# antbern/slamrs

Hardware: NVIDIA B200
Metric: particle_beam_updates_per_s (higher is better)
Workload: dtype f32 geometry, f64 weights, u16x2 hit-counter cells

## Files before the change

slamrs_b200/csrc/api.cu:

```cuda
#include "../../include/slamrs_gpu.h"

#include <cuda_runtime.h>
#include <math.h>
#include <stdio.h>
#include <stdlib.h>
#include <string.h>
#include <unistd.h>

#include <algorithm>
#include <new>
#include <string>
#include <vector>

#include "comm.h"
#include "kernels.cuh"

using namespace slamrs;

struct slamrs_gpu_handle {
    slamrs_gpu_config cfg{};
    int device = 0;
    int num_sms = 148;
    cudaStream_t stream = nullptr;
    cudaStream_t side_stream = nullptr;
// ... 362 lines not shown
        launch_publish_counters(h->stream, h->d_counters, h->h_counters);
        h->launches++;
    }
    CU_TRY(h, cudaStreamSynchronize(h->stream));
    CU_TRY(h, cudaGetLastError());
    h->counters_fresh = true;
    return SLAMRS_OK;
}

int loc_step_async(slamrs_gpu_handle* h, const OdomModel& od, bool caller) {
    cudaStream_t s = h->stream;
    if (h->profiling && h->prof_recorded == PROF_RING) {
        int prc = prof_flush(h);
        if (prc) return prc;
    }
    const int cur = h->cur, nxt = cur ^ 1;
    const ScanDevice scan = h->scan_external ? ScanDevice{h->ext_angle, h->ext_dist, h->ext_valid, h->n_beams, nullptr}
                                             : ScanDevice{h->d_angle, h->d_dist, h->d_valid, h->n_beams, nullptr};
    PROF_MARK(h, 0);
    launch_loc_step(s, h->geom, od, scan, h->d_pose[cur], h->d_results, h->n_total, caller ? h->d_z : nullptr, h->cfg.seed,
                    h->step, h->d_loc_terms, h->loc_outside, h->d_carry, h->d_counters);
    PROF_MARK(h, 1);
    PROF_MARK(h, 2);
    launch_weights(s, h->d_results, h->n_total, h->d_wnorm, h->d_cum, h->d_fold, (double)h->cfg.resample_threshold, h->d_counters);
    launch_resample_indices(s, h->d_results, h->d_cum, h->n_total, caller ? h->d_u : nullptr, h->cfg.seed, h->step, h->d_idx,
                            h->d_pose[nxt], 0, h->n_total, false, nullptr,
                            RayLists{nullptr, nullptr, nullptr, nullptr, nullptr, nullptr, 0u, 0u}, h->d_wnorm, h->d_carry,
                            h->d_counters);
    h->launches += 3;
    for (uint32_t m = 3; m < PROF_MARKS; ++m) PROF_MARK(h, m);
    if (h->profiling) h->prof_recorded++;
    CU_TRY(h, cudaGetLastError());
    h->cur = nxt;
    h->step++;
    h->counters_fresh = false;
    h->mirror_by_step = false;
    return SLAMRS_OK;
}

}

namespace {
template <typename T>
struct DevBuf {
    T* p = nullptr;
    cudaError_t alloc(size_t n) { return cudaMalloc(&p, sizeof(T) * (n ? n : 1)); }
    ~DevBuf() { cudaFree(p); }
};
int debug_device(int device) {
    int n = 0;
    if (cudaGetDeviceCount(&n) != cudaSuccess || n == 0) { cudaGetLastError(); return SLAMRS_E_NO_DEVICE; }
// ... 506 lines not shown
    const bool flag_pulls = h->world > 1 && fuse && half_items && h->boxed_copy && h->p2p_exchange;
    const uint32_t pull_epoch = flag_pulls ? (uint32_t)(h->step + 1ull) : 0u;
    const size_t n_zero = half_items ? 2 * (size_t)h->n_slots + 2 * (size_t)h->n_local : 0;
    PROF_MARK(h, 0);
    launch_motion_likelihood(s, h->geom, od, scan, h->d_pose[cur], h->d_slot[cur], h->defer ? h->d_alias : nullptr, h->d_cells, h->d_meta, h->cells_per_grid,
                             h->d_results, h->first, h->n_local, caller ? h->d_z : nullptr, h->cfg.seed, h->step, h->d_term_table, h->d_valid_list, h->d_n_valid,
                             h->d_carry, h->d_counters, h->p2p_exchange ? h->d_peer_results : nullptr, res_off, h->rank, h->world,
                             h->d_readers, (uint32_t)n_zero, h->match_on ? &h->match : nullptr, h->d_match_stats);
    h->launches += h->match_on ? 3 : 2;
    h->match_last_step = h->match_on;
    h->match_last_max_moves = h->match.max_moves;
    PROF_MARK(h, 1);
    if (h->world > 1) {
        if (h->p2p_exchange) {
            int brc = step_barrier(h);
            if (brc) return brc;
        } else {
            std::string err;
            if (comm_all_gather(h->comm, h->d_results + h->first, h->d_results, sizeof(ParticleResult) * h->n_local, s, &err))
                return fail(h, SLAMRS_E_NCCL, err);
        }
    }
    PROF_MARK(h, 2);
    launch_weights(s, h->d_results, h->n_total, h->d_wnorm, h->d_cum, h->d_fold, (double)h->cfg.resample_threshold, h->d_counters);
    RayLists ray{nullptr, nullptr, nullptr, nullptr, nullptr, nullptr, 0u, 0u};
    if (fuse) ray = RayLists{h->d_ray_items, h->d_ray_items + h->n_local, h->d_slot[cur], h->d_alias, h->d_readers, h->d_meta,
                             h->n_local, flag_pulls ? 1u : 0u};
    launch_resample_indices(s, h->d_results, h->d_cum, h->n_total, caller ? h->d_u : nullptr, h->cfg.seed, h->step,
                            h->d_idx, h->d_pose[nxt], h->first, h->n_local, !all_particles, h->d_alive, ray, h->d_wnorm, h->d_carry,
                            h->d_counters);
    if (all_particles) {
        launch_mark_alive(s, h->d_idx, h->n_total, h->first, h->n_local, true, h->d_alive, h->d_counters);
        h->launches++;
    }
    if (h->defer && !fuse) {
        if (all_particles)
            launch_materialize_list(s, nullptr, h->n_total, h->first, h->n_local, h->d_slot[cur], h->d_alias, h->d_cells,
                                    h->cells_per_grid, h->d_meta, h->d_bands, h->n_bands, h->d_mat_items, h->d_mat_leaders,
                                    h->d_mat_roots, h->d_counters);
        else
            launch_materialize_alive(s, h->d_alive, h->n_local, h->d_slot[cur], h->d_alias, h->d_cells, h->cells_per_grid,
                                     h->d_meta, h->d_bands, h->n_bands, h->d_mat_items, h->d_counters);
        h->launches++;
    }
    CU_TRY(h, cudaEventRecord(h->ev_indices, s));
    CU_TRY(h, cudaStreamWaitEvent(h->side_stream, h->ev_indices, 0));
    PlanArgs pa{};
    pa.results = h->d_results;
    pa.idx = h->d_idx;
    pa.n_total = h->n_total; pa.n_local = h->n_local; pa.rank = h->rank; pa.world = h->world;
    pa.slot_old = h->d_slot[cur]; pa.slot_new = h->d_slot[nxt];
    pa.keep = h->d_keep; pa.need = h->d_need; pa.free_list = h->d_free; pa.spare_list = h->d_spare;
    pa.n_spare_cap = h->n_spare;
    pa.copies = h->d_copies; pa.leaders = h->d_leaders;
    pa.cells = h->d_cells; pa.cells_per_grid = h->cells_per_grid;
    pa.peer_cells = h->d_peer_cells;
    pa.meta = h->d_meta; pa.peer_meta = h->d_peer_meta;
    pa.bands = h->d_bands; pa.peer_bands = h->d_peer_bands; pa.n_bands = h->n_bands;
    pa.counters = h->d_counters;
    pa.history = h->d_history;
    pa.step = h->step;
    pa.staged = plan_can_stage(h->n_local, h->n_spare);
    pa.alias_of = h->d_alias; pa.defer = h->defer;
    launch_plan(h->side_stream, pa);
    h->launches += 3;
    if (flag_pulls) {
        launch_pull(h->side_stream, h->d_copies, h->d_leaders, &h->d_counters->n_copies, &h->d_counters->n_leaders,
                    h->n_local, h->geom, h->d_counters, h->num_sms, pull_epoch, h->barrier_timeout_ns, h->d_meta, h->d_readers,
                    h->d_readers + h->n_slots);
        h->launches++;
    }
    CU_TRY(h, cudaEventRecord(h->ev_plan, h->side_stream));
    PROF_MARK(h, 3);
    if (h->defer && !fuse) {
        int mrc = materialize_copies(h, all_particles);
        if (mrc) return mrc;
    }
    PROF_MARK(h, 4);
    if (h->order_pending) {
        CU_TRY(h, cudaStreamWaitEvent(s, h->ev_sort, 0));
        h->order_pending = false;
    }
    CU_TRY(h, launch_ray_update(s, h->geom, scan, h->d_results, h->first, h->n_local, h->d_alive,
                                fuse ? h->d_ray_items : nullptr, fuse ? h->d_ray_items + h->n_local : nullptr,
                                fuse ? h->d_readers : nullptr,
                                fuse ? h->d_readers + h->n_slots : nullptr, h->d_readers + 2 * (size_t)h->n_slots, h->d_ray_xchg,
                                h->d_ray_spill, h->d_slot[cur],
                                h->d_cells, h->d_meta, h->d_bands, h->cells_per_grid, h->radius_cells, h->d_counters, &h->window_cells,
// ... 566 lines not shown
                                       uint64_t out_shape[4]) {
    if (!raw_weights || !out_idx || n == 0 || n > 0x7fffffffu || !(tau >= 0.0 && tau <= 1.0)) return SLAMRS_E_INVALID_ARG;
    int rc = debug_device(device);
    if (rc) return rc;
    DeviceGuard g(device < 0 ? 0 : device);
    DBG_CU(configure_kernels());
    DevBuf<ParticleResult> res;
    DevBuf<double> wn, cum, fold, u;
    DevBuf<uint32_t> idx;
    DevBuf<StepCounters> cnt;
    DBG_CU(res.alloc(n)); DBG_CU(wn.alloc(n)); DBG_CU(cum.alloc(n)); DBG_CU(fold.alloc(weights_scratch_doubles()));
    DBG_CU(u.alloc(1)); DBG_CU(idx.alloc(n)); DBG_CU(cnt.alloc(1));
    std::vector<ParticleResult> host(n);
    for (uint32_t i = 0; i < n; ++i) { host[i].weight = raw_weights[i]; host[i].x = host[i].y = host[i].theta = 0.0f; host[i].slot = 0; }
    DBG_CU(cudaMemcpy(res.p, host.data(), sizeof(ParticleResult) * (size_t)n, cudaMemcpyHostToDevice));
    DBG_CU(cudaMemcpy(u.p, &u01, sizeof(double), cudaMemcpyHostToDevice));
    DBG_CU(cudaMemset(cnt.p, 0, sizeof(StepCounters)));
    cudaEvent_t ev[3];
    for (auto& e : ev) DBG_CU(cudaEventCreate(&e));
    const int reps = out_us ? 20 : 1;
    float us[2] = {0.f, 0.f};
    for (int r = 0; r < reps; ++r) {
        cudaEventRecord(ev[0], nullptr);
        launch_weights(nullptr, res.p, n, wn.p, cum.p, fold.p, tau, cnt.p);
        cudaEventRecord(ev[1], nullptr);
        launch_resample_indices(nullptr, res.p, cum.p, n, u.p, 0, 0, idx.p, nullptr, 0, 0, false, nullptr,
                                RayLists{nullptr, nullptr, nullptr, nullptr, nullptr, nullptr, 0u, 0u}, wn.p, nullptr, cnt.p);
        cudaEventRecord(ev[2], nullptr);
        cudaError_t e = cudaDeviceSynchronize();
        if (e != cudaSuccess) { for (auto& x : ev) cudaEventDestroy(x); return fail(nullptr, SLAMRS_E_CUDA, cudaGetErrorString(e)); }
        float a = 0.f, b = 0.f;
        cudaEventElapsedTime(&a, ev[0], ev[1]); cudaEventElapsedTime(&b, ev[1], ev[2]);
        if (r > 0 || reps == 1) { us[0] += a * 1000.f; us[1] += b * 1000.f; }
    }
    for (auto& e : ev) cudaEventDestroy(e);
    if (out_us) { out_us[0] = us[0] / (float)(reps > 1 ? reps - 1 : 1); out_us[1] = us[1] / (float)(reps > 1 ? reps - 1 : 1); }
    StepCounters c;
    DBG_CU(cudaMemcpy(&c, cnt.p, sizeof(c), cudaMemcpyDeviceToHost));
    DBG_CU(cudaMemcpy(out_idx, idx.p, sizeof(uint32_t) * (size_t)n, cudaMemcpyDeviceToHost));
    if (out_norm) DBG_CU(cudaMemcpy(out_norm, wn.p, sizeof(double) * (size_t)n, cudaMemcpyDeviceToHost));
    if (out_cum) DBG_CU(cudaMemcpy(out_cum, cum.p, sizeof(double) * (size_t)n, cudaMemcpyDeviceToHost));
    if (out_max_particle) *out_max_particle = c.max_particle;
    if (out_us && getenv("SLAMRS_FOLD_TRACE_PRINT")) {
        long long tr[64];
        if (weights_trace(tr) == 0) {
            fprintf(stderr, "k_weights clock stamps (cycles from start):");
            for (int k = 0; k < 44; ++k) fprintf(stderr, " [%d]%lld", k, tr[k] ? tr[k] - tr[0] : -1);
            fprintf(stderr, "\n");
        }
    }
// ... 12 lines not shown
```

slamrs_b200/csrc/kernels.cuh:

```cuda
#pragma once
#include <cuda_runtime.h>
#include <stdint.h>
#include "slam_device.cuh"

namespace slamrs {

struct alignas(8) ParticleResult {
    double weight;
    float x, y, theta;
    int32_t slot;
};
static_assert(sizeof(ParticleResult) == 24, "ParticleResult is exchanged between GPUs as 24 bytes");

struct StepCounters {
    unsigned long long max_particle;
    unsigned long long n_copies;
    unsigned long long n_leaders;
    unsigned long long n_pulls;
    unsigned long long distinct;
    unsigned long long clamped;
    unsigned long long saturated;
    unsigned long long spilled;
    unsigned long long staging_short;
    long long est_slot;
// ... 115 lines not shown
                         uint32_t rank, uint32_t world, unsigned long long epoch, unsigned long long timeout_ns,
                         StepCounters* counters);
void launch_peer_goodbye(cudaStream_t stream, unsigned long long* const* peer_flags, unsigned long long* my_flags,
                         uint32_t rank, uint32_t world, unsigned long long timeout_ns, StepCounters* counters);

bool ray_update_can_fuse(const MapGeom& geom, uint32_t n_beams, size_t cells_per_grid, bool force_generic, int radius_cells);
size_t ray_spill_scratch_words(int num_sms);
size_t ray_half_xchg_bytes();
int ray_trace(unsigned long long* out18);
cudaError_t launch_ray_update(cudaStream_t stream, MapGeom geom, ScanDevice scan, const ParticleResult* results,
                              uint32_t first_particle, uint32_t n_local, const uint32_t* alive_list,
                              const RayItem* clones, const RayItem* owners, const uint32_t* readers, uint32_t* done,
                              uint32_t* xflag , void* xchg ,
                              uint32_t* spill_scratch,
                              const int32_t* slot_of, uint32_t* cells, SlotMeta* meta, uint32_t* bands,
                              size_t cells_per_grid, int radius_cells, StepCounters* counters,
                              uint64_t* window_cells, bool force_generic, int num_sms,
                              uint32_t* xdone ,

                              uint32_t signal_epoch );

struct WeightsShape { uint32_t cluster, threads, chunk; bool regs; };
WeightsShape weights_shape(uint32_t n_total);
void launch_weights(cudaStream_t stream, const ParticleResult* results, uint32_t n_total, double* w_norm,
                    double* cum, double* fold_scratch, double resample_tau, StepCounters* counters);
size_t weights_scratch_doubles();
int weights_trace(long long* out64);

void launch_resample_indices(cudaStream_t stream, const ParticleResult* results, const double* cum,
                             uint32_t n_total, const double* u01_caller, uint64_t seed, uint64_t step,
                             uint32_t* idx, float* pose_next, uint32_t first_particle, uint32_t n_local,
                             bool build_alive ,
                             uint32_t* alive_list, RayLists ray, const double* w_norm, double* carry ,
                             StepCounters* counters);

struct PlanArgs {
    const ParticleResult* results;
    const uint32_t* idx;
    uint32_t n_total, n_local, rank, world;
    const int32_t* slot_old;
    int32_t* slot_new;
    int32_t* keep;
    int32_t* need;
    int32_t* free_list;
    int32_t* spare_list;
    uint32_t n_spare_cap;
    CopyItem* copies;
    uint32_t* leaders;
    uint32_t* cells;
    size_t cells_per_grid;
    uint32_t* const* peer_cells;
    SlotMeta* meta;
    SlotMeta* const* peer_meta;
    uint32_t* bands;
    uint32_t* const* peer_bands;
    uint32_t n_bands;
    StepCounters* counters;
// ... 74 lines not shown
```

slamrs_b200/csrc/kernels_resample.cu:

```cuda
#include "kernels_common.cuh"

namespace slamrs {


constexpr int W_CLUSTER = 8;

constexpr uint32_t FOLD_HEADS_PER_CTA = 32;
constexpr uint32_t FOLD_HEADS_MAX = FOLD_HEADS_PER_CTA * W_CLUSTER;
constexpr uint32_t FOLD_STAGE = 2048;
constexpr int FOLD_MAX_ROUNDS = 4;
constexpr int FOLD_MARGIN_BITS = 40;
constexpr int FOLD_LREG = 16;
constexpr int FOLD_THREADS = 512;
constexpr int FOLD_GENERIC_THREADS = 1024;
constexpr uint32_t FOLD_MAX_CHUNKS = FOLD_GENERIC_THREADS * W_CLUSTER;

struct FoldTd {
    double d0, d1;
    uint32_t qc;
};
template <int LREG>
struct FoldRec {
    double d0, d1;
    uint32_t q_prev;
// ... 263 lines not shown
                if (C == 1u) sh.total = s;
                else for (uint32_t r = 0; r < C; ++r) *cluster.map_shared_rank(&sh.total, r) = s;
            }
        }
        FOLD_STAMP(tb + 5);
        __syncthreads();
        if (tid < C) {
            if (C == 1u) sh.cta_bad[0] = sh.bad;
            else cluster.map_shared_rank(&sh.cta_bad[0], tid)[crank] = sh.bad;
        }
        fold_sync(cluster, C);
        FOLD_STAMP(tb + 6);
        uint32_t bad = 0xffffffffu;
        for (uint32_t r = 0; r < C; ++r) bad = min(bad, sh.cta_bad[r]);
        if (bad == 0xffffffffu) { *total = sh.total; return true; }
        t0 = bad;
        s0 = __ldcg(&sout[bad - 1u]);
        a_base = __ldcg(&ain[bad]);
        if (!f64_finite(s0)) return false;
    }
    return false;
}

template <int LREG, int THREADS>
__global__ void __launch_bounds__(THREADS)
k_weights(const ParticleResult* __restrict__ results, uint32_t n, double* __restrict__ w_norm,
          double* __restrict__ cum, double* __restrict__ fold_scratch, double resample_tau, StepCounters* counters) {
    cg::cluster_group cluster = cg::this_cluster();
    const uint32_t crank = cluster.block_rank(), C = cluster.num_blocks();
    __shared__ FoldShared<LREG> sh;
    __shared__ double s_sq[W_CLUSTER];
    __shared__ long long s_key[32];
    __shared__ uint32_t s_arg[32];
    __shared__ long long s_ckey[W_CLUSTER];
    __shared__ uint32_t s_carg[W_CLUSTER];
    __shared__ double s_seq[2];
    pdl_launch_dependents();
    pdl_wait();
    FOLD_STAMP(0);
    const uint32_t gt = crank * THREADS + threadIdx.x;
    const uint32_t L = LREG ? (uint32_t)LREG : (n + C * THREADS - 1u) / (C * THREADS);
    const uint32_t lo = min(n, gt * L), hi = min(n, lo + L), cnt = hi - lo;

    extern __shared__ __align__(16) double s_tile[];
    auto tile_of = [](uint32_t e) { return e + e / (uint32_t)(LREG ? LREG : 1); };
    const uint32_t warp_e0 = (threadIdx.x >> 5) * 32u * (uint32_t)(LREG ? LREG : 1);
    const uint32_t cta_e0 = crank * THREADS * (uint32_t)(LREG ? LREG : 1);
    double v[LREG ? LREG : 1];
    double part = 0.0;
    bool all_zero = true;
// ... 58 lines not shown
        }
        __syncthreads();
        sum = s_seq[0];
    }

    double sqpart = 0.0;
    long long best_key = (long long)0x8000000000000000ull;
    uint32_t best_i = 0;
    bool have = false;
    all_zero = true;
    auto norm_one = [&](uint32_t j, double x) {
        const double w = __ddiv_rn(x, sum);
        if (LREG) s_tile[threadIdx.x * (LREG + 1) + j] = w; else w_norm[lo + j] = w;
        sqpart = __dadd_rn(sqpart, __dmul_rn(w, w));
        all_zero = all_zero && w == 0.0;
        const long long k = total_order_key(w);
        if (!have || k >= best_key) { best_key = k; best_i = lo + j; have = true; }
        return w;
    };
    if (LREG) {
#pragma unroll
        for (int j = 0; j < (LREG ? LREG : 1); ++j) v[j] = (uint32_t)j < cnt ? norm_one(j, v[j]) : 0.0;
        flush_tile(w_norm);
    } else {
        for (uint32_t j = 0; j < cnt; ++j) norm_one(j, results[lo + j].weight);
    }
    FOLD_STAMP(4);
    double cta_sq;
    const double sq_offset = block_excl_scan_f64(sqpart, sh.warp_f64, &cta_sq);

    const int lane = threadIdx.x & 31, wid = threadIdx.x >> 5;
    auto argmax_warp = [&]() {
#pragma unroll
        for (int o = 16; o > 0; o >>= 1) {
            const long long okey = __shfl_down_sync(0xffffffffu, best_key, o);
            const uint32_t oi = __shfl_down_sync(0xffffffffu, best_i, o);
            const bool ohave = __shfl_down_sync(0xffffffffu, (int)have, o) != 0;
            if (ohave && (!have || okey > best_key || (okey == best_key && oi > best_i))) { best_key = okey; best_i = oi; have = true; }
        }
    };
    argmax_warp();
    if (lane == 0) { s_key[wid] = best_key; s_arg[wid] = have ? best_i : 0xffffffffu; }
    __syncthreads();
    if (wid == 0) {
        have = lane < (THREADS >> 5) && s_arg[lane] != 0xffffffffu;
        best_key = have ? s_key[lane] : (long long)0x8000000000000000ull;
        best_i = have ? s_arg[lane] : 0u;
        argmax_warp();
        if (lane == 0) {
            if (C == 1u) { s_ckey[0] = best_key; s_carg[0] = have ? best_i : 0xffffffffu; s_sq[0] = cta_sq; }
            else {
                cluster.map_shared_rank(&s_ckey[0], 0)[crank] = best_key;
                cluster.map_shared_rank(&s_carg[0], 0)[crank] = have ? best_i : 0xffffffffu;
                cluster.map_shared_rank(&s_sq[0], 0)[crank] = cta_sq;
            }
        }
    }
    FOLD_STAMP(5);

    if (ok) {
        double c_in, c_out, c_total;
        ok = exact_left_fold<LREG>(cluster, sh, n, L, cnt, all_zero, __ddiv_rn(r_in, sum), __ddiv_rn(r_out, sum), v,
                                   [&](uint32_t j, double s) { if (LREG) s_tile[threadIdx.x * (LREG + 1) + j] = s; else cum[lo + j] = s; },
                                   [&](uint32_t i) { return __ldcg(&w_norm[i]); }, true, fold_scratch, &c_in, &c_out, &c_total,
                                   &info_cum, 16);
        if (!ok) info_cum.fallback = 1u;
        else if (LREG) flush_tile(cum);
    } else {
        info_cum.rounds = 0u; info_cum.heads = 0u; info_cum.fallback = 1u;
    }
    FOLD_STAMP(6);
    if (!ok) {
        fold_sync(cluster, C);
        if (gt == 0) {
            double c = 0.0;
            for (uint32_t i = 0; i < n; ++i) { const double w = __ldcg(&w_norm[i]); c = i ? __dadd_rn(c, w) : w; cum[i] = c; }
        }
// ... 2 lines not shown

    FoldInfo info_sq = {0u, 0u, 0u};
    double sq_exact = 0.0;
    if (resample_tau > 0.0) {
        double q_in = sq_offset;
        if (C > 1u) {
            if (threadIdx.x < C) cluster.map_shared_rank(&sh.cta_part[0], threadIdx.x)[crank] = cta_sq;
            cluster.sync();
            q_in = 0.0;
            for (uint32_t r = 0; r < crank; ++r) q_in = __dadd_rn(q_in, sh.cta_part[r]);
            q_in = __dadd_rn(q_in, sq_offset);
        }
        if (LREG) {
#pragma unroll
            for (int j = 0; j < (LREG ? LREG : 1); ++j) v[j] = __dmul_rn(v[j], v[j]);
        }
        double q_lo, q_hi;
        const bool sq_ok = exact_left_fold<LREG>(cluster, sh, n, L, cnt, all_zero, q_in, __dadd_rn(q_in, sqpart), v,
                                                 [](uint32_t, double) {},
                                                 [&](uint32_t i) { const double w = __ldcg(&w_norm[i]); return __dmul_rn(w, w); },
                                                 false, fold_scratch, &q_lo, &q_hi, &sq_exact, &info_sq, 24);
        if (!sq_ok) {
            info_sq.fallback = 1u;
            if (gt == 0) {
                double s = 0.0;
                for (uint32_t i = 0; i < n; ++i) { const double w = __ldcg(&w_norm[i]); s = __dadd_rn(s, __dmul_rn(w, w)); }
                sq_exact = s;
            }
        }
    }
    if (gt == 0) {
        long long bk = 0; uint32_t bi = 0; bool h = false;
        for (uint32_t r = 0; r < C; ++r) {
            if (s_carg[r] == 0xffffffffu) continue;
            if (!h || s_ckey[r] > bk || (s_ckey[r] == bk && s_carg[r] > bi)) { bk = s_ckey[r]; bi = s_carg[r]; h = true; }
        }
        counters->max_particle = bi;
        counters->sum = sum;
        double sq = sq_exact;
        if (!(resample_tau > 0.0)) {
            sq = 0.0;
            for (uint32_t r = 0; r < C; ++r) sq = __dadd_rn(sq, s_sq[r]);
        }
        counters->n_eff = __ddiv_rn(1.0, sq);
        counters->do_resample = (resample_tau > 0.0 && !(__ddiv_rn(1.0, sq) < __dmul_rn(resample_tau, (double)n))) ? 0ull : 1ull;
        counters->fold_rounds = (unsigned long long)max(max(info_sum.rounds, info_cum.rounds), info_sq.rounds);
        counters->fold_heads = (unsigned long long)max(max(info_sum.heads, info_cum.heads), info_sq.heads);
        counters->fold_fallback = (unsigned long long)(info_sum.fallback | (info_cum.fallback << 1) | (info_sq.fallback << 2));
    }
    FOLD_STAMP(7);
}

static size_t weights_tile_bytes() { return sizeof(double) * FOLD_THREADS * (FOLD_LREG + 1); }
WeightsShape weights_shape(uint32_t n_total) {
    uint32_t c = 1u;
    while (c < (uint32_t)W_CLUSTER && (uint64_t)c * FOLD_THREADS * FOLD_LREG < n_total) c <<= 1;
    WeightsShape s;
    s.cluster = c;
    s.regs = (uint64_t)c * FOLD_THREADS * FOLD_LREG >= n_total;
    s.threads = s.regs ? (uint32_t)FOLD_THREADS : (uint32_t)FOLD_GENERIC_THREADS;
    s.chunk = s.regs ? (uint32_t)FOLD_LREG : (uint32_t)(((uint64_t)n_total + c * s.threads - 1u) / (c * s.threads));
    return s;
}
void launch_weights(cudaStream_t stream, const ParticleResult* results, uint32_t n_total, double* w_norm,
                    double* cum, double* fold_scratch, double resample_tau, StepCounters* counters) {
    const WeightsShape shape = weights_shape(n_total);
    const uint32_t c = shape.cluster;
    const bool regs = shape.regs;
    cudaLaunchConfig_t cfg = {};
    cfg.gridDim = dim3(c, 1, 1);
    cfg.blockDim = dim3(shape.threads, 1, 1);
    cfg.dynamicSmemBytes = regs ? weights_tile_bytes() : 0;
    cfg.stream = stream;
    cudaLaunchAttribute attr[2];
    attr[0].id = cudaLaunchAttributeClusterDimension;
    attr[0].val.clusterDim.x = c; attr[0].val.clusterDim.y = 1; attr[0].val.clusterDim.z = 1;
    attr[1].id = cudaLaunchAttributeProgrammaticStreamSerialization;
    attr[1].val.programmaticStreamSerializationAllowed = 1;
    cfg.attrs = attr;
    cfg.numAttrs = 2;
    if (regs) cudaLaunchKernelEx(&cfg, k_weights<FOLD_LREG, FOLD_THREADS>, results, n_total, w_norm, cum, fold_scratch, resample_tau, counters);
    else cudaLaunchKernelEx(&cfg, k_weights<0, FOLD_GENERIC_THREADS>, results, n_total, w_norm, cum, fold_scratch, resample_tau, counters);
}
size_t weights_scratch_doubles() { return 2u * FOLD_MAX_CHUNKS; }
int weights_trace(long long* out64) {
#ifdef SLAMRS_FOLD_TRACE
    return (int)cudaMemcpyFromSymbol(out64, g_fold_trace, sizeof(long long) * 64);
#else
    (void)out64;
    return -1;
#endif
}


__device__ __forceinline__ double resample_threshold(uint32_t n, double U, uint32_t m0) {
    const double num = (double)n;
    const double r = __ddiv_rn(__dmul_rn(U, 1.0), num);
    return __dadd_rn(r, __ddiv_rn(__dmul_rn(__dsub_rn((double)(m0 + 1u), 1.0), 1.0), num));
}
__device__ __forceinline__ uint32_t first_not_below(const double* __restrict__ cum, uint32_t lo, uint32_t hi, double u) {
    while (lo < hi) {
        const uint32_t mid = lo + ((hi - lo) >> 1);
        if (u > cum[mid]) lo = mid + 1; else hi = mid;
    }
    return lo;
}

constexpr uint32_t RS_COARSE = 2048;

__global__ void __launch_bounds__(256)
k_resample_indices(const ParticleResult* __restrict__ results, const double* __restrict__ cum, uint32_t n,
                   const double* __restrict__ u01_caller, uint64_t seed, uint64_t step, uint32_t* __restrict__ idx,
                   float* __restrict__ pose_next, uint32_t first_particle, uint32_t n_local, bool build_alive,
                   uint32_t* __restrict__ alive_list, RayLists ray, const double* __restrict__ w_norm,
                   double* __restrict__ carry, StepCounters* counters) {
    __shared__ double s_coarse[RS_COARSE];
    pdl_wait();
    const bool resample = counters->do_resample != 0ull;
    const uint32_t stride = (n + RS_COARSE - 1u) / RS_COARSE;
    const uint32_t n_coarse = (n + stride - 1u) / stride;
    for (uint32_t j = threadIdx.x; j < n_coarse; j += blockDim.x) s_coarse[j] = cum[min(n, (j + 1u) * stride) - 1u];
    __syncthreads();
    const uint32_t m0 = blockIdx.x * blockDim.x + threadIdx.x;
    const double U = u01_caller ? *u01_caller : slamrs_stream::resample_uniform(seed, step);
    const int lane = threadIdx.x & 31;
    auto source_of = [&](uint32_t m, bool* ran_off) {
        const double u = resample_threshold(n, U, m);
        const uint32_t blk = first_not_below(s_coarse, 0u, n_coarse, u);
        *ran_off = blk >= n_coarse;
        if (blk >= n_coarse) return n - 1u;
        return first_not_below(cum, blk * stride, min(n, (blk + 1u) * stride) - 1u, u);
    };
    bool ran_off = false;
    uint32_t src_idx = 0xffffffffu;
    if (m0 < n) {
        if (resample) src_idx = source_of(m0, &ran_off); else src_idx = m0;
        if (carry != nullptr) carry[m0] = w_norm[m0];
        if (m0 == 0u) counters->carry_active = resample ? 0ull : 1ull;
        if (ran_off) atomicAdd(&counters->clamped, 1ull);
        idx[m0] = src_idx;
        const ParticleResult src = results[src_idx];
        if (m0 >= first_particle && m0 < first_particle + n_local) {
            float* q = pose_next + 3 * (size_t)(m0 - first_particle);
            q[0] = src.x; q[1] = src.y; q[2] = src.theta;
        }
        if ((unsigned long long)m0 == counters->max_particle) {
            counters->est_pose[0] = src.x; counters->est_pose[1] = src.y; counters->est_pose[2] = src.theta;
        }
    }
    if (!build_alive) return;
    uint32_t prev = __shfl_up_sync(0xffffffffu, src_idx, 1);
    if (lane == 0 && m0 > 0 && m0 < n) {
        bool dummy;
        prev = resample ? source_of(m0 - 1u, &dummy) : m0 - 1u;
    }
    const bool alive = m0 < n && (m0 == 0 || prev != src_idx) && src_idx >= first_particle &&
                       src_idx < first_particle + n_local;
    if (ray.clones == nullptr) {
        const unsigned mask = __ballot_sync(0xffffffffu, alive);
        if (mask) {
            const int leader = __ffs(mask) - 1;
            unsigned long long base = 0;
            if (lane == leader) base = atomicAdd(&counters->n_alive, (unsigned long long)__popc(mask));
            base = __shfl_sync(0xffffffffu, base, leader);
            if (alive) alive_list[base + __popc(mask & ((1u << lane) - 1u))] = src_idx - first_particle;
        }
        return;
    }
    RayItem it{0u, 0, 0, 0, 0, 0u};
    bool clone = false, remote = false;
    if (alive && ray.mark_remote != 0u) {
        const uint32_t end = first_particle + n_local;
        remote = !(m0 >= first_particle && m0 < end);
        if (!remote && end < n) {
            bool dummy;
            remote = (resample ? source_of(end, &dummy) : end) == src_idx;
        }
    }
    if (alive) {
        it.pad = remote ? 1u : 0u;
        it.particle = src_idx - first_particle;
        it.slot = ray.slot_of[it.particle];
        it.root = ray.alias_of[it.slot];
        clone = it.root != it.slot;
        if (clone) {
            atomicAdd(&ray.readers[it.root], 2u);
            ray.alias_of[it.slot] = it.slot;
            const SlotMeta old = ray.meta[it.slot];
            if (old.x1 > old.x0 && old.y1 > old.y0) { it.old_y0 = old.y0; it.old_y1 = old.y1; }
            SlotMeta src = ray.meta[it.root];
            src.pad0 = 0;
            ray.meta[it.slot] = src;
        }
    }
    const unsigned mcr = __ballot_sync(0xffffffffu, alive && clone && remote), mcl = __ballot_sync(0xffffffffu, alive && clone && !remote);
    const unsigned mor = __ballot_sync(0xffffffffu, alive && !clone && remote), mol = __ballot_sync(0xffffffffu, alive && !clone && !remote);
    unsigned long long bcr = 0, bcl = 0, bor = 0, bol = 0;
    if (lane == 0) {
        const unsigned mc = mcr | mcl, all = mc | mor | mol;
        if (all) atomicAdd(&counters->n_alive, (unsigned long long)__popc(all));
        if (mc) {
            atomicAdd(&counters->n_mat, (unsigned long long)__popc(mc));
            atomicAdd(&counters->n_mat_leaders, (unsigned long long)__popc(mc));
        }
        if (mcr) bcr = atomicAdd(&counters->ray_items_front, (unsigned long long)__popc(mcr));
        if (mcl) bcl = atomicAdd(&counters->ray_items_front_local, (unsigned long long)__popc(mcl));
        if (mor) bor = atomicAdd(&counters->ray_items_back, (unsigned long long)__popc(mor));
        if (mol) bol = atomicAdd(&counters->ray_items_back_local, (unsigned long long)__popc(mol));
    }
    bcr = __shfl_sync(0xffffffffu, bcr, 0); bcl = __shfl_sync(0xffffffffu, bcl, 0);
    bor = __shfl_sync(0xffffffffu, bor, 0); bol = __shfl_sync(0xffffffffu, bol, 0);
    const unsigned below = (1u << lane) - 1u;
    if (alive && clone && remote) ray.clones[bcr + __popc(mcr & below)] = it;
    if (alive && clone && !remote) ray.clones[ray.n_local - 1u - (bcl + __popc(mcl & below))] = it;
    if (alive && !clone && remote) ray.owners[bor + __popc(mor & below)] = it;
    if (alive && !clone && !remote) ray.owners[ray.n_local - 1u - (bol + __popc(mol & below))] = it;
}

void launch_resample_indices(cudaStream_t stream, const ParticleResult* results, const double* cum,
                             uint32_t n_total, const double* u01_caller, uint64_t seed, uint64_t step,
                             uint32_t* idx, float* pose_next, uint32_t first_particle, uint32_t n_local,
                             bool build_alive, uint32_t* alive_list, RayLists ray, const double* w_norm, double* carry,
                             StepCounters* counters) {
    launch_pdl(k_resample_indices, dim3((n_total + 255) / 256), dim3(256), 0, stream, results, cum, n_total, u01_caller, seed, step, idx,
               pose_next, first_particle, n_local, build_alive, alive_list, ray, w_norm, carry, counters);
}

__global__ void __launch_bounds__(256)
k_mark_alive(const uint32_t* __restrict__ idx, uint32_t n_total, uint32_t first_particle, uint32_t n_local,
             bool all_particles, uint32_t* __restrict__ alive_list, StepCounters* counters) {
    const uint32_t j = blockIdx.x * blockDim.x + threadIdx.x;
    bool alive = false;
    if (j < n_local) {
        if (all_particles) {
            alive = true;
        } else {
            const uint32_t v = first_particle + j;
            uint32_t lo = 0, hi = n_total;
            while (lo < hi) {
                const uint32_t mid = lo + ((hi - lo) >> 1);
                if (idx[mid] < v) lo = mid + 1; else hi = mid;
            }
            alive = lo < n_total && idx[lo] == v;
        }
    }
    const unsigned m = __ballot_sync(0xffffffffu, alive);
    if (m) {
        const int lane = threadIdx.x & 31, leader = __ffs(m) - 1;
// ... 375 lines not shown
```

Baseline: 15.50 billion.

## Fuse resample index generation into the clustered weights kernel

```diff
diff --git a/slamrs_b200/csrc/api.cu b/slamrs_b200/csrc/api.cu
--- a/slamrs_b200/csrc/api.cu
+++ b/slamrs_b200/csrc/api.cu
@@ -408,11 +408,10 @@
                     h->step, h->d_loc_terms, h->loc_outside, h->d_carry, h->d_counters);
     PROF_MARK(h, 1);
     PROF_MARK(h, 2);
-    launch_weights(s, h->d_results, h->n_total, h->d_wnorm, h->d_cum, h->d_fold, (double)h->cfg.resample_threshold, h->d_counters);
-    launch_resample_indices(s, h->d_results, h->d_cum, h->n_total, caller ? h->d_u : nullptr, h->cfg.seed, h->step, h->d_idx,
-                            h->d_pose[nxt], 0, h->n_total, false, nullptr,
-                            RayLists{nullptr, nullptr, nullptr, nullptr, nullptr, nullptr, 0u, 0u}, h->d_wnorm, h->d_carry,
-                            h->d_counters);
+    const ResampleArgs ra{caller ? h->d_u : nullptr, h->cfg.seed, h->step, h->d_idx, h->d_pose[nxt], 0, h->n_total, false, nullptr,
+                          RayLists{nullptr, nullptr, nullptr, nullptr, nullptr, nullptr, 0u, 0u}, h->d_carry};
+    launch_resample(s, h->d_results, h->n_total, h->d_wnorm, h->d_cum, h->d_fold, (double)h->cfg.resample_threshold, ra,
+                    h->d_counters, false);
     h->launches += 3;
     for (uint32_t m = 3; m < PROF_MARKS; ++m) PROF_MARK(h, m);
     if (h->profiling) h->prof_recorded++;
@@ -965,13 +964,13 @@
         }
     }
     PROF_MARK(h, 2);
-    launch_weights(s, h->d_results, h->n_total, h->d_wnorm, h->d_cum, h->d_fold, (double)h->cfg.resample_threshold, h->d_counters);
     RayLists ray{nullptr, nullptr, nullptr, nullptr, nullptr, nullptr, 0u, 0u};
     if (fuse) ray = RayLists{h->d_ray_items, h->d_ray_items + h->n_local, h->d_slot[cur], h->d_alias, h->d_readers, h->d_meta,
                              h->n_local, flag_pulls ? 1u : 0u};
-    launch_resample_indices(s, h->d_results, h->d_cum, h->n_total, caller ? h->d_u : nullptr, h->cfg.seed, h->step,
-                            h->d_idx, h->d_pose[nxt], h->first, h->n_local, !all_particles, h->d_alive, ray, h->d_wnorm, h->d_carry,
-                            h->d_counters);
+    const ResampleArgs ra{caller ? h->d_u : nullptr, h->cfg.seed, h->step, h->d_idx, h->d_pose[nxt], h->first, h->n_local,
+                          !all_particles, h->d_alive, ray, h->d_carry};
+    const bool fused = launch_resample(s, h->d_results, h->n_total, h->d_wnorm, h->d_cum, h->d_fold,
+                                       (double)h->cfg.resample_threshold, ra, h->d_counters);
     if (all_particles) {
         launch_mark_alive(s, h->d_idx, h->n_total, h->first, h->n_local, true, h->d_alive, h->d_counters);
         h->launches++;
@@ -1006,7 +1005,7 @@
     pa.staged = plan_can_stage(h->n_local, h->n_spare);
     pa.alias_of = h->d_alias; pa.defer = h->defer;
     launch_plan(h->side_stream, pa);
-    h->launches += 3;
+    h->launches += fused ? 2 : 3;
     if (flag_pulls) {
         launch_pull(h->side_stream, h->d_copies, h->d_leaders, &h->d_counters->n_copies, &h->d_counters->n_leaders,
                     h->n_local, h->geom, h->d_counters, h->num_sms, pull_epoch, h->barrier_timeout_ns, h->d_meta, h->d_readers,
@@ -1619,10 +1618,9 @@
     float us[2] = {0.f, 0.f};
     for (int r = 0; r < reps; ++r) {
         cudaEventRecord(ev[0], nullptr);
-        launch_weights(nullptr, res.p, n, wn.p, cum.p, fold.p, tau, cnt.p);
-        cudaEventRecord(ev[1], nullptr);
-        launch_resample_indices(nullptr, res.p, cum.p, n, u.p, 0, 0, idx.p, nullptr, 0, 0, false, nullptr,
-                                RayLists{nullptr, nullptr, nullptr, nullptr, nullptr, nullptr, 0u, 0u}, wn.p, nullptr, cnt.p);
+        const ResampleArgs ra{u.p, 0, 0, idx.p, nullptr, 0, 0, false, nullptr,
+                              RayLists{nullptr, nullptr, nullptr, nullptr, nullptr, nullptr, 0u, 0u}, nullptr};
+        if (launch_resample(nullptr, res.p, n, wn.p, cum.p, fold.p, tau, ra, cnt.p, true, ev[1])) cudaEventRecord(ev[1], nullptr);
         cudaEventRecord(ev[2], nullptr);
         cudaError_t e = cudaDeviceSynchronize();
         if (e != cudaSuccess) { for (auto& x : ev) cudaEventDestroy(x); return fail(nullptr, SLAMRS_E_CUDA, cudaGetErrorString(e)); }
diff --git a/slamrs_b200/csrc/kernels.cuh b/slamrs_b200/csrc/kernels.cuh
--- a/slamrs_b200/csrc/kernels.cuh
+++ b/slamrs_b200/csrc/kernels.cuh
@@ -161,17 +161,22 @@
 
 struct WeightsShape { uint32_t cluster, threads, chunk; bool regs; };
 WeightsShape weights_shape(uint32_t n_total);
-void launch_weights(cudaStream_t stream, const ParticleResult* results, uint32_t n_total, double* w_norm,
-                    double* cum, double* fold_scratch, double resample_tau, StepCounters* counters);
+struct ResampleArgs {
+    const double* u01_caller;
+    uint64_t seed, step;
+    uint32_t* idx;
+    float* pose_next;
+    uint32_t first_particle, n_local;
+    bool build_alive;
+    uint32_t* alive_list;
+    RayLists ray;
+    double* carry;
+};
+bool launch_resample(cudaStream_t stream, const ParticleResult* results, uint32_t n_total, double* w_norm, double* cum,
+                     double* fold_scratch, double resample_tau, const ResampleArgs& ra, StepCounters* counters,
+                     bool fuse_indices = true, cudaEvent_t split_event = nullptr);
 size_t weights_scratch_doubles();
 int weights_trace(long long* out64);
-
-void launch_resample_indices(cudaStream_t stream, const ParticleResult* results, const double* cum,
-                             uint32_t n_total, const double* u01_caller, uint64_t seed, uint64_t step,
-                             uint32_t* idx, float* pose_next, uint32_t first_particle, uint32_t n_local,
-                             bool build_alive ,
-                             uint32_t* alive_list, RayLists ray, const double* w_norm, double* carry ,
-                             StepCounters* counters);
 
 struct PlanArgs {
     const ParticleResult* results;
diff --git a/slamrs_b200/csrc/kernels_resample.cu b/slamrs_b200/csrc/kernels_resample.cu
--- a/slamrs_b200/csrc/kernels_resample.cu
+++ b/slamrs_b200/csrc/kernels_resample.cu
@@ -309,10 +309,187 @@
     return false;
 }
 
+
+__device__ __forceinline__ double resample_threshold(uint32_t n, double U, uint32_t m0) {
+    const double num = (double)n;
+    const double r = __ddiv_rn(__dmul_rn(U, 1.0), num);
+    return __dadd_rn(r, __ddiv_rn(__dmul_rn(__dsub_rn((double)(m0 + 1u), 1.0), 1.0), num));
+}
+template <typename Cum>
+__device__ __forceinline__ uint32_t first_not_below(Cum cum, uint32_t lo, uint32_t hi, double u) {
+    while (lo < hi) {
+        const uint32_t mid = lo + ((hi - lo) >> 1);
+        if (u > cum(mid)) lo = mid + 1; else hi = mid;
+    }
+    return lo;
+}
+
+__device__ __forceinline__ unsigned long long block_excl_scan_u64(unsigned long long v, unsigned long long* warp_tot ,
+                                                                  unsigned long long* total) {
+    const int lane = threadIdx.x & 31, wid = threadIdx.x >> 5, nw = (blockDim.x + 31) >> 5;
+    unsigned long long inc = v;
+#pragma unroll
+    for (int o = 1; o < 32; o <<= 1) {
+        const unsigned long long t = __shfl_up_sync(0xffffffffu, inc, o);
+        if (lane >= o) inc += t;
+    }
+    __syncthreads();
+    if (lane == 31) warp_tot[wid] = inc;
+    __syncthreads();
+    if (wid == 0) {
+        unsigned long long w = lane < nw ? warp_tot[lane] : 0ull;
+#pragma unroll
+        for (int o = 1; o < 32; o <<= 1) {
+            const unsigned long long t = __shfl_up_sync(0xffffffffu, w, o);
+            if (lane >= o) w += t;
+        }
+        if (lane == 31) warp_tot[32] = w;
+        warp_tot[lane] = w - (lane < nw ? warp_tot[lane] : 0ull);
+    }
+    __syncthreads();
+    *total = warp_tot[32];
+    return warp_tot[wid] + inc - v;
+}
+
+template <int M, typename Search>
+__device__ void resample_generation(const ParticleResult* __restrict__ results, uint32_t n, const ResampleArgs& a,
+                                    bool resample, unsigned long long max_particle, Search search,
+                                    unsigned long long* warp_tot , unsigned long long* s_base ,
+                                    StepCounters* counters) {
+    const uint32_t T = blockDim.x, tid = threadIdx.x;
+    const uint32_t span0 = blockIdx.x * (uint32_t)M * T;
+    const double U = a.u01_caller ? *a.u01_caller : slamrs_stream::resample_uniform(a.seed, a.step);
+    auto source_of = [&](uint32_t m, uint32_t lo, bool near, bool* ran_off) {
+        if (!resample) { *ran_off = false; return m; }
+        const uint32_t i = search(resample_threshold(n, U, m), lo, near);
+        *ran_off = i >= n;
+        return i >= n ? n - 1u : i;
+    };
+    const uint32_t m_first = span0 + (uint32_t)M * tid;
+    unsigned long long n_off = 0;
+    uint32_t lo = 0;
+#pragma unroll 1
+    for (int j = 0; j < M; ++j) {
+        const uint32_t m = m_first + (uint32_t)j;
+        if (m >= n) break;
+        bool off;
+        lo = source_of(m, lo, j > 0, &off);
+        n_off += off ? 1ull : 0ull;
+        a.idx[m] = lo;
+    }
+    if (n_off) atomicAdd(&counters->clamped, n_off);
+    if (m_first == 0u) counters->carry_active = resample ? 0ull : 1ull;
+    __syncthreads();
+    constexpr int G = M < 4 ? M : 4;
+#pragma unroll 1
+    for (int k0 = 0; k0 < M; k0 += G) {
+        uint32_t src[G];
+        ParticleResult r[G];
+#pragma unroll
+        for (int g = 0; g < G; ++g) {
+            const uint32_t m = span0 + (uint32_t)(k0 + g) * T + tid;
+            src[g] = m < n ? a.idx[m] : 0u;
+        }
+#pragma unroll
+        for (int g = 0; g < G; ++g) r[g] = results[src[g]];
+#pragma unroll
+        for (int g = 0; g < G; ++g) {
+            const uint32_t m = span0 + (uint32_t)(k0 + g) * T + tid;
+            if (m >= n) continue;
+            if (a.pose_next != nullptr && m >= a.first_particle && m < a.first_particle + a.n_local) {
+                float* q = a.pose_next + 3 * (size_t)(m - a.first_particle);
+                q[0] = r[g].x; q[1] = r[g].y; q[2] = r[g].theta;
+            }
+            if ((unsigned long long)m == max_particle) {
+                counters->est_pose[0] = r[g].x; counters->est_pose[1] = r[g].y; counters->est_pose[2] = r[g].theta;
+            }
+        }
+    }
+    if (!a.build_alive) return;
+    const uint32_t first = a.first_particle, end = first + a.n_local;
+    uint32_t alive_bits = 0, remote_bits = 0, clone_bits = 0;
+    unsigned long long cnt = 0;
+#pragma unroll 1
+    for (int k = 0; k < M; ++k) {
+        const uint32_t m = span0 + (uint32_t)k * T + tid;
+        if (m >= n) break;
+        const uint32_t src = a.idx[m];
+        if (src < first || src >= end) continue;
+        if (m > 0u) {
+            bool dummy;
+            const uint32_t p = m > span0 ? a.idx[m - 1u] : source_of(m - 1u, 0u, false, &dummy);
+            if (p == src) continue;
+        }
+        alive_bits |= 1u << k;
+        if (a.ray.clones == nullptr) { cnt += 1ull; continue; }
+        bool remote = false;
+        if (a.ray.mark_remote != 0u) {
+            remote = !(m >= first && m < end);
+            if (!remote && end < n) { bool dummy; remote = source_of(end, 0u, false, &dummy) == src; }
+        }
+        const int32_t slot = a.ray.slot_of[src - first];
+        const bool clone = a.ray.alias_of[slot] != slot;
+        remote_bits |= remote ? 1u << k : 0u;
+        clone_bits |= clone ? 1u << k : 0u;
+        cnt += 1ull << (16 * ((clone ? 0 : 2) + (remote ? 0 : 1)));
+    }
+    unsigned long long cta_cnt;
+    unsigned long long off = block_excl_scan_u64(cnt, warp_tot, &cta_cnt);
+    if (tid == 0) {
+        if (a.ray.clones == nullptr) {
+            if (cta_cnt) s_base[0] = atomicAdd(&counters->n_alive, cta_cnt);
+        } else {
+            auto f = [&](int c) { return (cta_cnt >> (16 * c)) & 0xffffull; };
+            const unsigned long long mc = f(0) + f(1), all = mc + f(2) + f(3);
+            if (all) atomicAdd(&counters->n_alive, all);
+            if (mc) {
+                atomicAdd(&counters->n_mat, mc);
+                atomicAdd(&counters->n_mat_leaders, mc);
+            }
+            if (f(0)) s_base[0] = atomicAdd(&counters->ray_items_front, f(0));
+            if (f(1)) s_base[1] = atomicAdd(&counters->ray_items_front_local, f(1));
+            if (f(2)) s_base[2] = atomicAdd(&counters->ray_items_back, f(2));
+            if (f(3)) s_base[3] = atomicAdd(&counters->ray_items_back_local, f(3));
+        }
+    }
+    __syncthreads();
+    const RayLists& ray = a.ray;
+    unsigned long long k_alive = s_base[0] + off;
+    while (alive_bits != 0u) {
+        const int k = __ffs(alive_bits) - 1;
+        alive_bits &= alive_bits - 1u;
+        const uint32_t src = a.idx[span0 + (uint32_t)k * T + tid];
+        if (ray.clones == nullptr) { a.alive_list[k_alive++] = src - first; continue; }
+        const bool clone = (clone_bits >> k) & 1u, remote = (remote_bits >> k) & 1u;
+        RayItem it{0u, 0, 0, 0, 0, 0u};
+        it.pad = remote ? 1u : 0u;
+        it.particle = src - first;
+        it.slot = ray.slot_of[it.particle];
+        it.root = ray.alias_of[it.slot];
+        if (clone) {
+            atomicAdd(&ray.readers[it.root], 2u);
+            ray.alias_of[it.slot] = it.slot;
+            const SlotMeta old = ray.meta[it.slot];
+            if (old.x1 > old.x0 && old.y1 > old.y0) { it.old_y0 = old.y0; it.old_y1 = old.y1; }
+            SlotMeta sm = ray.meta[it.root];
+            sm.pad0 = 0;
+            ray.meta[it.slot] = sm;
+        }
+        const int c = (clone ? 0 : 2) + (remote ? 0 : 1);
+        const unsigned long long kk = s_base[c] + ((off >> (16 * c)) & 0xffffull);
+        off += 1ull << (16 * c);
+        if (c == 0) ray.clones[kk] = it;
+        else if (c == 1) ray.clones[ray.n_local - 1u - kk] = it;
+        else if (c == 2) ray.owners[kk] = it;
+        else ray.owners[ray.n_local - 1u - kk] = it;
+    }
+}
+
 template <int LREG, int THREADS>
 __global__ void __launch_bounds__(THREADS)
 k_weights(const ParticleResult* __restrict__ results, uint32_t n, double* __restrict__ w_norm,
-          double* __restrict__ cum, double* __restrict__ fold_scratch, double resample_tau, StepCounters* counters) {
+          double* __restrict__ cum, double* __restrict__ fold_scratch, double resample_tau, StepCounters* counters,
+          ResampleArgs ra, bool fuse) {
     cg::cluster_group cluster = cg::this_cluster();
     const uint32_t crank = cluster.block_rank(), C = cluster.num_blocks();
     __shared__ FoldShared<LREG> sh;
@@ -417,6 +594,7 @@
 #pragma unroll
         for (int j = 0; j < (LREG ? LREG : 1); ++j) v[j] = (uint32_t)j < cnt ? norm_one(j, v[j]) : 0.0;
         flush_tile(w_norm);
+        if (fuse && ra.carry != nullptr) flush_tile(ra.carry);
     } else {
         for (uint32_t j = 0; j < cnt; ++j) norm_one(j, results[lo + j].weight);
     }
@@ -442,12 +620,15 @@
         best_key = have ? s_key[lane] : (long long)0x8000000000000000ull;
         best_i = have ? s_arg[lane] : 0u;
         argmax_warp();
-        if (lane == 0) {
+        best_key = __shfl_sync(0xffffffffu, best_key, 0);
+        best_i = __shfl_sync(0xffffffffu, best_i, 0);
+        have = __shfl_sync(0xffffffffu, (int)have, 0) != 0;
+        if (lane < C) {
             if (C == 1u) { s_ckey[0] = best_key; s_carg[0] = have ? best_i : 0xffffffffu; s_sq[0] = cta_sq; }
             else {
-                cluster.map_shared_rank(&s_ckey[0], 0)[crank] = best_key;
-                cluster.map_shared_rank(&s_carg[0], 0)[crank] = have ? best_i : 0xffffffffu;
-                cluster.map_shared_rank(&s_sq[0], 0)[crank] = cta_sq;
+                cluster.map_shared_rank(&s_ckey[0], lane)[crank] = best_key;
+                cluster.map_shared_rank(&s_carg[0], lane)[crank] = have ? best_i : 0xffffffffu;
+                if (lane == 0) cluster.map_shared_rank(&s_sq[0], 0)[crank] = cta_sq;
             }
         }
     }
@@ -496,19 +677,22 @@
                                                  false, fold_scratch, &q_lo, &q_hi, &sq_exact, &info_sq, 24);
         if (!sq_ok) {
             info_sq.fallback = 1u;
-            if (gt == 0) {
+            if (threadIdx.x == 0) {
                 double s = 0.0;
                 for (uint32_t i = 0; i < n; ++i) { const double w = __ldcg(&w_norm[i]); s = __dadd_rn(s, __dmul_rn(w, w)); }
-                sq_exact = s;
-            }
-        }
-    }
+                s_seq[1] = s;
+            }
+            __syncthreads();
+            sq_exact = s_seq[1];
+        }
+    }
+    long long bk = 0; uint32_t bi = 0; bool h = false;
+    for (uint32_t r = 0; r < C; ++r) {
+        if (s_carg[r] == 0xffffffffu) continue;
+        if (!h || s_ckey[r] > bk || (s_ckey[r] == bk && s_carg[r] > bi)) { bk = s_ckey[r]; bi = s_carg[r]; h = true; }
+    }
+    const bool resample = !(resample_tau > 0.0 && !(__ddiv_rn(1.0, sq_exact) < __dmul_rn(resample_tau, (double)n)));
     if (gt == 0) {
-        long long bk = 0; uint32_t bi = 0; bool h = false;
-        for (uint32_t r = 0; r < C; ++r) {
-            if (s_carg[r] == 0xffffffffu) continue;
-            if (!h || s_ckey[r] > bk || (s_ckey[r] == bk && s_carg[r] > bi)) { bk = s_ckey[r]; bi = s_carg[r]; h = true; }
-        }
         counters->max_particle = bi;
         counters->sum = sum;
         double sq = sq_exact;
@@ -517,12 +701,35 @@
             for (uint32_t r = 0; r < C; ++r) sq = __dadd_rn(sq, s_sq[r]);
         }
         counters->n_eff = __ddiv_rn(1.0, sq);
-        counters->do_resample = (resample_tau > 0.0 && !(__ddiv_rn(1.0, sq) < __dmul_rn(resample_tau, (double)n))) ? 0ull : 1ull;
+        counters->do_resample = resample ? 1ull : 0ull;
         counters->fold_rounds = (unsigned long long)max(max(info_sum.rounds, info_cum.rounds), info_sq.rounds);
         counters->fold_heads = (unsigned long long)max(max(info_sum.heads, info_cum.heads), info_sq.heads);
         counters->fold_fallback = (unsigned long long)(info_sum.fallback | (info_cum.fallback << 1) | (info_sq.fallback << 2));
     }
     FOLD_STAMP(7);
+    if constexpr (LREG != 0) if (fuse) {
+        constexpr uint32_t SPAN = THREADS * LREG;
+        __shared__ unsigned long long s_wtot[33], s_base[4];
+        auto cum_at = [&](uint32_t i) -> double {
+            if (!ok) return __ldcg(&cum[i]);
+            const uint32_t r = i / SPAN, e = tile_of(i % SPAN);
+            if (r == crank) return s_tile[e];
+            return cluster.map_shared_rank(s_tile, r)[e];
+        };
+        auto search = [&](double u, uint32_t lo, bool near) {
+            uint32_t hi = n;
+            if (near) {
+                for (uint32_t step = 1u, b = lo; b < n; step <<= 1) {
+                    if (!(u > cum_at(b))) { hi = b; break; }
+                    lo = b + 1u; b = lo + step;
+                }
+            }
+            return first_not_below(cum_at, lo, hi, u);
+        };
+        resample_generation<LREG>(results, n, ra, resample, (unsigned long long)bi, search, s_wtot, s_base, counters);
+        if (C > 1u) cluster.sync();
+        FOLD_STAMP(32);
+    }
 }
 
 static size_t weights_tile_bytes() { return sizeof(double) * FOLD_THREADS * (FOLD_LREG + 1); }
@@ -536,11 +743,36 @@
     s.chunk = s.regs ? (uint32_t)FOLD_LREG : (uint32_t)(((uint64_t)n_total + c * s.threads - 1u) / (c * s.threads));
     return s;
 }
-void launch_weights(cudaStream_t stream, const ParticleResult* results, uint32_t n_total, double* w_norm,
-                    double* cum, double* fold_scratch, double resample_tau, StepCounters* counters) {
+constexpr uint32_t RS_COARSE = 2048;
+
+__global__ void __launch_bounds__(256)
+k_resample_indices(const ParticleResult* __restrict__ results, const double* __restrict__ cum, uint32_t n,
+                   const double* __restrict__ w_norm, StepCounters* counters, ResampleArgs ra) {
+    __shared__ double s_coarse[RS_COARSE];
+    __shared__ unsigned long long s_wtot[33], s_base[4];
+    pdl_wait();
+    const bool resample = counters->do_resample != 0ull;
+    const uint32_t stride = (n + RS_COARSE - 1u) / RS_COARSE;
+    const uint32_t n_coarse = (n + stride - 1u) / stride;
+    for (uint32_t j = threadIdx.x; j < n_coarse; j += blockDim.x) s_coarse[j] = cum[min(n, (j + 1u) * stride) - 1u];
+    __syncthreads();
+    const uint32_t m0 = blockIdx.x * blockDim.x + threadIdx.x;
+    auto search = [&](double u, uint32_t, bool) {
+        const uint32_t blk = first_not_below([&](uint32_t i) { return s_coarse[i]; }, 0u, n_coarse, u);
+        if (blk >= n_coarse) return n;
+        return first_not_below([&](uint32_t i) { return cum[i]; }, blk * stride, min(n, (blk + 1u) * stride) - 1u, u);
+    };
+    if (m0 < n && ra.carry != nullptr) ra.carry[m0] = w_norm[m0];
+    resample_generation<1>(results, n, ra, resample, counters->max_particle, search, s_wtot, s_base, counters);
+}
+
+bool launch_resample(cudaStream_t stream, const ParticleResult* results, uint32_t n_total, double* w_norm, double* cum,
+                     double* fold_scratch, double resample_tau, const ResampleArgs& ra, StepCounters* counters,
+                     bool fuse_indices, cudaEvent_t split_event) {
     const WeightsShape shape = weights_shape(n_total);
     const uint32_t c = shape.cluster;
     const bool regs = shape.regs;
+    const bool fuse = regs && fuse_indices;
     cudaLaunchConfig_t cfg = {};
     cfg.gridDim = dim3(c, 1, 1);
     cfg.blockDim = dim3(shape.threads, 1, 1);
@@ -553,8 +785,17 @@
     attr[1].val.programmaticStreamSerializationAllowed = 1;
     cfg.attrs = attr;
     cfg.numAttrs = 2;
-    if (regs) cudaLaunchKernelEx(&cfg, k_weights<FOLD_LREG, FOLD_THREADS>, results, n_total, w_norm, cum, fold_scratch, resample_tau, counters);
-    else cudaLaunchKernelEx(&cfg, k_weights<0, FOLD_GENERIC_THREADS>, results, n_total, w_norm, cum, fold_scratch, resample_tau, counters);
+    if (regs)
+        cudaLaunchKernelEx(&cfg, k_weights<FOLD_LREG, FOLD_THREADS>, results, n_total, w_norm, cum, fold_scratch, resample_tau,
+                           counters, ra, fuse);
+    else
+        cudaLaunchKernelEx(&cfg, k_weights<0, FOLD_GENERIC_THREADS>, results, n_total, w_norm, cum, fold_scratch, resample_tau,
+                           counters, ra, false);
+    if (fuse) return true;
+    if (split_event != nullptr) cudaEventRecord(split_event, stream);
+    launch_pdl(k_resample_indices, dim3((n_total + 255) / 256), dim3(256), 0, stream, results, (const double*)cum, n_total,
+               (const double*)w_norm, counters, ra);
+    return false;
 }
 size_t weights_scratch_doubles() { return 2u * FOLD_MAX_CHUNKS; }
 int weights_trace(long long* out64) {
@@ -564,140 +805,6 @@
     (void)out64;
     return -1;
 #endif
-}
-
-
-__device__ __forceinline__ double resample_threshold(uint32_t n, double U, uint32_t m0) {
-    const double num = (double)n;
-    const double r = __ddiv_rn(__dmul_rn(U, 1.0), num);
-    return __dadd_rn(r, __ddiv_rn(__dmul_rn(__dsub_rn((double)(m0 + 1u), 1.0), 1.0), num));
-}
-__device__ __forceinline__ uint32_t first_not_below(const double* __restrict__ cum, uint32_t lo, uint32_t hi, double u) {
-    while (lo < hi) {
-        const uint32_t mid = lo + ((hi - lo) >> 1);
-        if (u > cum[mid]) lo = mid + 1; else hi = mid;
-    }
-    return lo;
-}
-
-constexpr uint32_t RS_COARSE = 2048;
-
-__global__ void __launch_bounds__(256)
-k_resample_indices(const ParticleResult* __restrict__ results, const double* __restrict__ cum, uint32_t n,
-                   const double* __restrict__ u01_caller, uint64_t seed, uint64_t step, uint32_t* __restrict__ idx,
-                   float* __restrict__ pose_next, uint32_t first_particle, uint32_t n_local, bool build_alive,
-                   uint32_t* __restrict__ alive_list, RayLists ray, const double* __restrict__ w_norm,
-                   double* __restrict__ carry, StepCounters* counters) {
-    __shared__ double s_coarse[RS_COARSE];
-    pdl_wait();
-    const bool resample = counters->do_resample != 0ull;
-    const uint32_t stride = (n + RS_COARSE - 1u) / RS_COARSE;
-    const uint32_t n_coarse = (n + stride - 1u) / stride;
-    for (uint32_t j = threadIdx.x; j < n_coarse; j += blockDim.x) s_coarse[j] = cum[min(n, (j + 1u) * stride) - 1u];
-    __syncthreads();
-    const uint32_t m0 = blockIdx.x * blockDim.x + threadIdx.x;
-    const double U = u01_caller ? *u01_caller : slamrs_stream::resample_uniform(seed, step);
-    const int lane = threadIdx.x & 31;
-    auto source_of = [&](uint32_t m, bool* ran_off) {
-        const double u = resample_threshold(n, U, m);
-        const uint32_t blk = first_not_below(s_coarse, 0u, n_coarse, u);
-        *ran_off = blk >= n_coarse;
-        if (blk >= n_coarse) return n - 1u;
-        return first_not_below(cum, blk * stride, min(n, (blk + 1u) * stride) - 1u, u);
-    };
-    bool ran_off = false;
-    uint32_t src_idx = 0xffffffffu;
-    if (m0 < n) {
-        if (resample) src_idx = source_of(m0, &ran_off); else src_idx = m0;
-        if (carry != nullptr) carry[m0] = w_norm[m0];
-        if (m0 == 0u) counters->carry_active = resample ? 0ull : 1ull;
-        if (ran_off) atomicAdd(&counters->clamped, 1ull);
-        idx[m0] = src_idx;
-        const ParticleResult src = results[src_idx];
-        if (m0 >= first_particle && m0 < first_particle + n_local) {
-            float* q = pose_next + 3 * (size_t)(m0 - first_particle);
-            q[0] = src.x; q[1] = src.y; q[2] = src.theta;
-        }
-        if ((unsigned long long)m0 == counters->max_particle) {
-            counters->est_pose[0] = src.x; counters->est_pose[1] = src.y; counters->est_pose[2] = src.theta;
-        }
-    }
-    if (!build_alive) return;
-    uint32_t prev = __shfl_up_sync(0xffffffffu, src_idx, 1);
-    if (lane == 0 && m0 > 0 && m0 < n) {
-        bool dummy;
-        prev = resample ? source_of(m0 - 1u, &dummy) : m0 - 1u;
-    }
-    const bool alive = m0 < n && (m0 == 0 || prev != src_idx) && src_idx >= first_particle &&
-                       src_idx < first_particle + n_local;
-    if (ray.clones == nullptr) {
-        const unsigned mask = __ballot_sync(0xffffffffu, alive);
-        if (mask) {
-            const int leader = __ffs(mask) - 1;
-            unsigned long long base = 0;
-            if (lane == leader) base = atomicAdd(&counters->n_alive, (unsigned long long)__popc(mask));
-            base = __shfl_sync(0xffffffffu, base, leader);
-            if (alive) alive_list[base + __popc(mask & ((1u << lane) - 1u))] = src_idx - first_particle;
-        }
-        return;
-    }
-    RayItem it{0u, 0, 0, 0, 0, 0u};
-    bool clone = false, remote = false;
-    if (alive && ray.mark_remote != 0u) {
-        const uint32_t end = first_particle + n_local;
-        remote = !(m0 >= first_particle && m0 < end);
-        if (!remote && end < n) {
-            bool dummy;
-            remote = (resample ? source_of(end, &dummy) : end) == src_idx;
-        }
-    }
-    if (alive) {
-        it.pad = remote ? 1u : 0u;
-        it.particle = src_idx - first_particle;
-        it.slot = ray.slot_of[it.particle];
-        it.root = ray.alias_of[it.slot];
-        clone = it.root != it.slot;
-        if (clone) {
-            atomicAdd(&ray.readers[it.root], 2u);
-            ray.alias_of[it.slot] = it.slot;
-            const SlotMeta old = ray.meta[it.slot];
-            if (old.x1 > old.x0 && old.y1 > old.y0) { it.old_y0 = old.y0; it.old_y1 = old.y1; }
-            SlotMeta src = ray.meta[it.root];
-            src.pad0 = 0;
-            ray.meta[it.slot] = src;
-        }
-    }
-    const unsigned mcr = __ballot_sync(0xffffffffu, alive && clone && remote), mcl = __ballot_sync(0xffffffffu, alive && clone && !remote);
-    const unsigned mor = __ballot_sync(0xffffffffu, alive && !clone && remote), mol = __ballot_sync(0xffffffffu, alive && !clone && !remote);
-    unsigned long long bcr = 0, bcl = 0, bor = 0, bol = 0;
-    if (lane == 0) {
-        const unsigned mc = mcr | mcl, all = mc | mor | mol;
-        if (all) atomicAdd(&counters->n_alive, (unsigned long long)__popc(all));
-        if (mc) {
-            atomicAdd(&counters->n_mat, (unsigned long long)__popc(mc));
-            atomicAdd(&counters->n_mat_leaders, (unsigned long long)__popc(mc));
-        }
-        if (mcr) bcr = atomicAdd(&counters->ray_items_front, (unsigned long long)__popc(mcr));
-        if (mcl) bcl = atomicAdd(&counters->ray_items_front_local, (unsigned long long)__popc(mcl));
-        if (mor) bor = atomicAdd(&counters->ray_items_back, (unsigned long long)__popc(mor));
-        if (mol) bol = atomicAdd(&counters->ray_items_back_local, (unsigned long long)__popc(mol));
-    }
-    bcr = __shfl_sync(0xffffffffu, bcr, 0); bcl = __shfl_sync(0xffffffffu, bcl, 0);
-    bor = __shfl_sync(0xffffffffu, bor, 0); bol = __shfl_sync(0xffffffffu, bol, 0);
-    const unsigned below = (1u << lane) - 1u;
-    if (alive && clone && remote) ray.clones[bcr + __popc(mcr & below)] = it;
-    if (alive && clone && !remote) ray.clones[ray.n_local - 1u - (bcl + __popc(mcl & below))] = it;
-    if (alive && !clone && remote) ray.owners[bor + __popc(mor & below)] = it;
-    if (alive && !clone && !remote) ray.owners[ray.n_local - 1u - (bol + __popc(mol & below))] = it;
-}
-
-void launch_resample_indices(cudaStream_t stream, const ParticleResult* results, const double* cum,
-                             uint32_t n_total, const double* u01_caller, uint64_t seed, uint64_t step,
-                             uint32_t* idx, float* pose_next, uint32_t first_particle, uint32_t n_local,
-                             bool build_alive, uint32_t* alive_list, RayLists ray, const double* w_norm, double* carry,
-                             StepCounters* counters) {
-    launch_pdl(k_resample_indices, dim3((n_total + 255) / 256), dim3(256), 0, stream, results, cum, n_total, u01_caller, seed, step, idx,
-               pose_next, first_particle, n_local, build_alive, alive_list, ray, w_norm, carry, counters);
 }
 
 __global__ void __launch_bounds__(256)
```

Result: slower. 12.64 billion (median of 6 runs) (-18.5%).
